# ZLkanyo009/Yolo-compression-and-deployment-in-FPGA

Measured on AMD Instinct MI355X. Metric: images/sec slim_yolo_v2 int8 416x416, higher is better.
Workload: dtype int8; 1 GPU; slim_yolo_v2_q_bf int8, batch 64 per GPU, 416x416, 2 classes, conf 0.01; global_batch=64, parallelism=batch-shard x1, streams_per_gpu=4, ring_workgroups_per_launch=128, input=f32, input_batches_rotated=4

## Files before the change

yolo-compression-and-deployment-in-fpga_amd/csrc/conv3x3_ring.hip:

```cpp
#include "y355_common.h"
#ifndef Y355_RING_XCD_SHARE
#define Y355_RING_XCD_SHARE 1
#endif
#include <type_traits>
#include <hip/hip_ext.h>
#include <cstdlib>
#ifndef Y355_DIAG
#define Y355_DIAG 0
#endif
#ifndef Y355_DIAG12
#define Y355_DIAG12 (Y355_DIAG == 1 || Y355_DIAG == 2)
#endif
#ifndef Y355_RING_PF
#define Y355_RING_PF 4
#endif

__device__ __forceinline__ void rglds16(const void *g, void *lds) {
    __builtin_amdgcn_global_load_lds((const __attribute__((address_space(1))) void *)g,
                                     (__attribute__((address_space(3))) void *)lds, 16, 0, 0);
}
template <int N>
__device__ __forceinline__ void rwait_vmcnt() {
    static_assert(N >= 0, "vmcnt");
    asm volatile("s_waitcnt vmcnt(%0)" ::"n"(N > 63 ? 63 : N) : "memory");
}

constexpr float RMAGIC = 12582912.0f, RQLO = 12582785.0f, RQHI = 12583039.0f;
__device__ __forceinline__ float rvmax(float a, float b) {
    float d;
    asm("v_max_f32 %0, %1, %2" : "=v"(d) : "v"(a), "v"(b));
    return d;
}
__device__ __forceinline__ float rvmax3(float a, float b, float c) {
    float d;
    asm("v_max3_f32 %0, %1, %2, %3" : "=v"(d) : "v"(a), "v"(b), "v"(c));
    return d;
}
__device__ __forceinline__ float rvmin3(float a, float b, float c) {
    float d;
    asm("v_min3_f32 %0, %1, %2, %3" : "=v"(d) : "v"(a), "v"(b), "v"(c));
    return d;
}
template <int B>
__device__ __forceinline__ void rmax_to_byte(unsigned int &w, float a, float b) {
    if constexpr (B == 0)
        asm("v_max_f32_sdwa %0, %1, %2 dst_sel:BYTE_0 dst_unused:UNUSED_PAD src0_sel:DWORD src1_sel:DWORD" : "=v"(w) : "v"(a), "v"(b));
    else if constexpr (B == 1)
        asm("v_max_f32_sdwa %0, %1, %2 dst_sel:BYTE_1 dst_unused:UNUSED_PRESERVE src0_sel:DWORD src1_sel:DWORD" : "+v"(w) : "v"(a), "v"(b));
    else if constexpr (B == 2)
        asm("v_max_f32_sdwa %0, %1, %2 dst_sel:BYTE_2 dst_unused:UNUSED_PRESERVE src0_sel:DWORD src1_sel:DWORD" : "+v"(w) : "v"(a), "v"(b));
    else
        asm("v_max_f32_sdwa %0, %1, %2 dst_sel:BYTE_3 dst_unused:UNUSED_PRESERVE src0_sel:DWORD src1_sel:DWORD" : "+v"(w) : "v"(a), "v"(b));
}
__device__ __forceinline__ unsigned int rpack4(float a, float b, float c, float d) {
    const unsigned int ab = __builtin_amdgcn_perm(__float_as_uint(b), __float_as_uint(a), 0x0c0c0400u);
    const unsigned int cd = __builtin_amdgcn_perm(__float_as_uint(d), __float_as_uint(c), 0x04000c0cu);
    return ab | cd;
}

__device__ __forceinline__ void rwait_vmcnt_dyn(int n) {
#define RW_CASE(k) case k: asm volatile("s_waitcnt vmcnt(" #k ")" ::: "memory"); break;
    switch (n < 0 ? 0 : (n > 63 ? 63 : n)) {
        RW_CASE(0) RW_CASE(1) RW_CASE(2) RW_CASE(3) RW_CASE(4) RW_CASE(5) RW_CASE(6) RW_CASE(7) RW_CASE(8) RW_CASE(9)
        RW_CASE(10) RW_CASE(11) RW_CASE(12) RW_CASE(13) RW_CASE(14) RW_CASE(15) RW_CASE(16) RW_CASE(17) RW_CASE(18)
        RW_CASE(19) RW_CASE(20) RW_CASE(21) RW_CASE(22) RW_CASE(23) RW_CASE(24) RW_CASE(25) RW_CASE(26) RW_CASE(27)
        RW_CASE(28) RW_CASE(29) RW_CASE(30) RW_CASE(31) RW_CASE(32) RW_CASE(33) RW_CASE(34) RW_CASE(35) RW_CASE(36)
        RW_CASE(37) RW_CASE(38) RW_CASE(39) RW_CASE(40) RW_CASE(41) RW_CASE(42) RW_CASE(43) RW_CASE(44) RW_CASE(45)
        RW_CASE(46) RW_CASE(47) RW_CASE(48) RW_CASE(49) RW_CASE(50) RW_CASE(51) RW_CASE(52) RW_CASE(53) RW_CASE(54)
        RW_CASE(55) RW_CASE(56) RW_CASE(57) RW_CASE(58) RW_CASE(59) RW_CASE(60) RW_CASE(61) RW_CASE(62) RW_CASE(63)
    }
#undef RW_CASE
}

constexpr int ring_sp(int lo, int hi, int ppw, bool prev) {
    int n = 0;
    for (int u = lo; u <= hi; ++u) {
        if (u < 0 && !prev) continue;
        const int t = ((u % 9) + 9) % 9;
        if (t >= 1 && t <= ppw) ++n;
    }
    return n;
}

template <int CIN, int BN, int TH, int TW, bool POOL, int WM, int WN, int PF, bool ROLL, bool DIRECT_REQ, bool FPE = false>
__global__ __launch_bounds__(WM * WN * 64, (WM * WN == 4) ? 2 : 1) void conv3x3_i8_ring_kernel(const ConvParams p, const int total_tiles) {
    constexpr int NW = WM * WN;
    constexpr int NTHR = NW * 64;
    constexpr int NCH = CIN / 64, SPC = 9, KS = NCH * SPC;
    constexpr int PW = TW + 2, PH = TH + 2;
    constexpr int PWL = (PW + 7) / 8 * 8;
    constexpr int NPIX = PH * PWL;
    constexpr int BM = TH * TW;
    constexpr int MT_TOT = (BM + 15) / 16;
    constexpr int MT = (MT_TOT + WM - 1) / WM;
    constexpr int NT = BN / 16 / WN;
    constexpr int SLABB = (NPIX * 64 + 1023) / 1024 * 1024;
    constexpr int NPIECE = SLABB / 1024;
    constexpr int PPW = (NPIECE + NW - 1) / NW;
    constexpr int WB = (BN / 16) * 1024;
    constexpr int NFR = BN / 16;
    constexpr int WPW = (NFR + NW - 1) / NW;
    constexpr int WSLOTS = PF + 2;
    constexpr int OFF_W = 2 * SLABB;
    constexpr int OFF_DUMMY = OFF_W + WSLOTS * WB;
    constexpr int OFF_BIAS = OFF_DUMMY + 1024;
    constexpr int SROWS = POOL ? MT * WM * 4 : MT * WM * 16;
    constexpr int SSTR = BN + 16;
    constexpr int OROWS = POOL ? BM / 4 : BM;
    constexpr bool DIRECT = DIRECT_REQ && (SROWS * SSTR > SLABB);
    constexpr int NPASS = (!DIRECT && SROWS * SSTR > SLABB) ? 2 : 1;
    constexpr int RP = SROWS / NPASS;
    constexpr int CG = BN / 16;
    constexpr int NITP = (RP * CG + NTHR - 1) / NTHR;
    constexpr int NIT = DIRECT ? (POOL ? MT : MT * 4) : NPASS * NITP;
    static_assert(CIN % 64 == 0 && NT == 4, "64-channel chunks, four n-tiles per wave");
    static_assert(PPW <= 8 && PF >= 2 && PF <= 8, "slab pieces go out at t = 1..PPW");
    static_assert(!(FPE && (DIRECT_REQ || ROLL)), "the fp32 epilogue is written for the staged path and the unrolled chunk loop");
    static_assert(DIRECT || (RP * SSTR <= SLABB && MT % NPASS == 0), "staging fits the dead slot");
    constexpr int UNRC = ROLL ? 1 : NCH;
    constexpr bool STATIC = !ROLL && KS % WSLOTS == 0 && NCH % 2 == 0;
    extern __shared__ __attribute__((aligned(16))) char smem[];

    const int tid = threadIdx.x;
    const int lane = tid & 63;
    const int wave = __builtin_amdgcn_readfirstlane(tid >> 6);
    const int wm = wave / WN, wn = wave % WN;
    const int li = lane & 15, g = lane >> 4;
    const int H = p.H, W = p.W;

    static_assert((NW * 16) % PWL == 0 && NPIX % 16 == 0, "slab pieces step by whole patch rows");
    constexpr int PSTEP = NW * 16 / PWL;
    const int pix0 = wave * 16 + (lane >> 2);
    const int ppy0 = pix0 / PWL, ppx0 = min(pix0 % PWL, PW - 1);
    const int pwithin = ((lane & 3) ^ ((lane >> 3) & 3)) << 4;
    auto decode = [&](int tile, int &b, int &y0, int &x0, int &nb) {
        if (p.xcd_share_log2 > 0) {
            const int gs = 8 << p.xcd_share_log2;
            if (tile < (total_tiles & ~(gs - 1))) {
                const int j = tile & (gs - 1);
                tile = (tile & ~(gs - 1)) | ((j & 7) << p.xcd_share_log2) | (j >> 3);
            }
        }
        nb = tile % p.nblk;
        tile /= p.nblk;
        x0 = (tile % p.tiles_x) * TW;
        tile /= p.tiles_x;
        y0 = (tile % p.tiles_y) * TH;
        b = tile / p.tiles_y;
    };
    auto issue_slab_piece = [&](int b, int y0, int x0, int c, int slot, int j) {
        const int q = wave + NW * j;
        const int8_t *inb = p.in + (size_t)b * (H + 2) * (W + 2) * CIN + c * 64;
        const int gy = min(y0 + ppy0 + j * PSTEP, H + 1), gx = min(x0 + ppx0, W + 1);
        const int8_t *src = inb + ((size_t)gy * (W + 2) + gx) * CIN + pwithin;
        char *dst = (q < NPIECE) ? smem + slot * SLABB + q * 1024 : smem + OFF_DUMMY;
        rglds16(src, dst);
    };
    auto issue_w = [&](int nb, int ks, int slot) {
#pragma unroll
        for (int j = 0; j < WPW; ++j) {
            const int f = wave + NW * j;
            const bool ok = NFR % NW == 0 || f < NFR;
            const int8_t *src = p.w + ((size_t)(nb * KS + ks) * NFR + (ok ? f : 0)) * 1024 + lane * 16;
            char *dst = ok ? smem + OFF_W + slot * WB + f * 1024 : smem + OFF_DUMMY;
            rglds16(src, dst);
        }
    };
    auto wrap = [](int s) { return s >= WSLOTS ? s - WSLOTS : s; };
// ... 39 lines not shown
    for (int k = 0; k <= PF; ++k) {
        if (k < KS) issue_w(nb, k, k);
        else issue_w(nb, k - KS, k);
    }
    pstamp(1);
    const Requant rq = p.rq;
    unsigned int nsat = 0;
    bool first = true;

    for (;;) {
        int ntile = tile + gridDim.x;
        const bool more = ntile < total_tiles;
        if (!more) ntile = tile;
        int b2, y2, x2, nb2;
        decode(ntile, b2, y2, x2, nb2);
        int abase[MT][3];
        {
            int li_a = li, g_a = g;
            asm volatile("" : "+v"(li_a), "+v"(g_a));
#pragma unroll
            for (int m = 0; m < MT; ++m) {
                int row = (wm * MT + m) * 16 + li_a;
                row = min(row, BM - 1);
                int oy, ox;
                if constexpr (POOL) {
                    const int w = row >> 2, r = row & 3;
                    oy = 2 * (w / (TW / 2)) + (r >> 1);
                    ox = 2 * (w % (TW / 2)) + (r & 1);
                } else {
                    oy = row / TW;
                    ox = row % TW;
                }
#pragma unroll
                for (int dx = 0; dx < 3; ++dx)
                    abase[m][dx] = (oy * PWL + ox + dx) * 64 + ((g_a ^ (((ox + dx) >> 1) & 3)) << 4);
            }
        }

        v4i acc[MT][NT];
        if constexpr (!FPE) {
#pragma unroll
            for (int m = 0; m < MT; ++m)
#pragma unroll
                for (int t = 0; t < NT; ++t) acc[m][t] = (v4i){0, 0, 0, 0};
        }

        v4i bfb[2][NT];
        v4i afp[2];
        if (first) rwait_vmcnt<PF * WPW>();
        else rwait_vmcnt<PF * WPW + ring_sp(-PF, -1, PPW, true) + NIT>();
        __builtin_amdgcn_s_barrier();
        pstamp(first ? 2 : 6);
        if constexpr (FPE) {
            const v4i bv = *(const v4i *)(smem + OFF_BIAS + (nb * BN + wn * (NT * 16) + li * NT) * 4);
#pragma unroll
            for (int m = 0; m < MT; ++m)
#pragma unroll
                for (int t = 0; t < NT; ++t) acc[m][t] = (v4i){bv[t], bv[t], bv[t], bv[t]};
        }
        {
            const char *wb0 = smem + OFF_W + (STATIC ? 0 : wq) * WB + (wn * NT) * 1024 + lane * 16;
#pragma unroll
            for (int tt = 0; tt < NT; ++tt) bfb[0][tt] = *(const v4i *)(wb0 + tt * 1024);
        }
#pragma unroll UNRC
        for (int c = 0; c < NCH; ++c) {
            const int slc = STATIC ? (c & 1) : sl;
            const int soff = slc * SLABB;
            const bool lastc = (c + 1 == NCH);
#pragma unroll
            for (int t = 0; t < SPC; ++t) {
                const int s_idx = c * SPC + t;
                {
                    constexpr int n_slab = (9 - PPW) * WPW;
                    const bool fine = Y355_DIAG12 && first && c == (NCH > 1 ? 1 : 0);
                    if (fine) stamp();
                    if constexpr (ROLL) {
                        const int n0f = (PF - 1) * WPW + ring_sp(t - PF + 1, t - 1, PPW, false);
                        int n0l = (PF - 1) * WPW + ring_sp(t - PF + 1, t - 1, PPW, true) + (t < PF ? NIT : 0);
                        int nr = (PF - 1) * WPW + ring_sp(9 + t - PF + 1, 9 + t - 1, PPW, true);
                        if (t == 0) {
                            if (n_slab + NIT < n0l) n0l = n_slab + NIT;
                            if (n_slab < nr) nr = n_slab;
                        }
                        if (c == 0) {
                            if (first) rwait_vmcnt_dyn(n0f);
                            else rwait_vmcnt_dyn(n0l);
                        } else {
                            rwait_vmcnt_dyn(nr);
                        }
                    } else {
                        const int lo = s_idx - PF + 1, hi = s_idx - 1;
                        int n_first = (PF - 1) * WPW + ring_sp(lo, hi, PPW, false);
                        int n_later = (PF - 1) * WPW + ring_sp(lo, hi, PPW, true) + (s_idx < PF ? NIT : 0);
                        if (t == 0) {
                            if (c > 0 && n_slab < n_first) n_first = n_slab;
                            const int n_slab2 = n_slab + (c == 0 ? NIT : 0);
                            if (n_slab2 < n_later) n_later = n_slab2;
                        }
                        if (n_first == n_later) rwait_vmcnt_dyn(n_later);
                        else if (first) rwait_vmcnt_dyn(n_first);
                        else rwait_vmcnt_dyn(n_later);
                    }
                    if (fine) stamp();
                }
                __builtin_amdgcn_s_barrier();
                if (Y355_DIAG12 && first && c == (NCH > 1 ? 1 : 0)) stamp();
// ... 142 lines not shown
                            }
                            const int qq = y355_requant_fast(v, bias[t], rq);
                            const int q = y355_clamp8<int>(qq);
                            nsat += (srow < OROWS && oy0 + srow / OTW < Ho && ox0 + srow % OTW < Wo && q != qq) ? 1u : 0u;
                            w |= (unsigned int)(q & 0xff) << (8 * t);
                        }
                        const int oy = oy0 + srow / OTW, ox = ox0 + srow % OTW;
                        int8_t *dst = outb + ((size_t)(oy + halo) * (Wo + 2 * halo) + ox + halo) * p.cstride + ncol;
                        if (!(srow < OROWS && oy < Ho && ox < Wo)) dst = p.sink + tid * 4;
                        *(unsigned int *)dst = w;
                        __builtin_amdgcn_sched_barrier(0);
                    }
            } else {
            asm volatile("s_waitcnt lgkmcnt(0)" ::: "memory");
            __builtin_amdgcn_s_barrier();
#pragma unroll
            for (int ps = 0; ps < NPASS; ++ps) {
                if (ps > 0) {
                    asm volatile("s_waitcnt lgkmcnt(0)" ::: "memory");
                    __builtin_amdgcn_s_barrier();
                }
                constexpr int MH = MT / NPASS;
                constexpr int RPMT = POOL ? 4 : 16;
                auto stage = [&](auto clampc) {
                    constexpr bool CL = decltype(clampc)::value;
#pragma unroll
                    for (int mm = 0; mm < MH; ++mm) {
                        const int m = ps * MH + mm;
#pragma unroll
                        for (int r = 0; r < RPM; ++r) {
                            const int lrow = POOL ? (wm * MH + mm) * 4 + g : (wm * MH + mm) * 16 + 4 * g + r;
                            unsigned int w = 0;
                            float yq[NT], ypos[NT], yneg[NT];
#pragma unroll
                            for (int t = 0; t < NT; ++t) {
                                int v;
                                if constexpr (POOL) {
                                    const v4i a = acc[m][t];
                                    v = max(max(a[0], a[1]), max(a[2], a[3]));
                                } else {
                                    v = acc[m][t][r];
                                }
                                if constexpr (FPE) {
                                    if constexpr (CL) asm volatile("" : "+v"(v));
                                    yq[t] = requantf(v, t, ypos[t], yneg[t]);
                                } else {
                                    const int qq = requant(v, t);
                                    const int q = y355_clamp8<int>(qq);
                                    satx += (unsigned int)(q ^ qq);
                                    w |= (unsigned int)(q & 0xff) << (8 * t);
                                }
                            }
                            if constexpr (FPE) {
                                static_assert(!FPE || NT == 4, "the fp32 epilogue packs four channels per lane and row");
                                if constexpr (CL) {
                                    float yc[NT];
#pragma unroll
                                    for (int t = 0; t < NT; ++t) yc[t] = __builtin_amdgcn_fmed3f(rvmax(ypos[t], yneg[t]), RQLO, RQHI);
                                    w = rpack4(yc[0], yc[1], yc[2], yc[3]);
                                } else {
                                    ymx = rvmax3(rvmax3(ymx, ypos[0], ypos[1]), ypos[2], ypos[3]);
                                    ymn = rvmin3(rvmin3(ymn, yneg[0], yneg[1]), yneg[2], yneg[3]);
                                    rmax_to_byte<0>(w, ypos[0], yneg[0]);
                                    rmax_to_byte<1>(w, ypos[1], yneg[1]);
                                    rmax_to_byte<2>(w, ypos[2], yneg[2]);
                                    rmax_to_byte<3>(w, ypos[3], yneg[3]);
                                }
                            }
                            *(unsigned int *)(stg + lrow * SSTR + ncol) = w;
                            if constexpr (FPE) __builtin_amdgcn_sched_barrier(0);
                        }
                    }
                };
                stage(std::false_type{});
                if constexpr (FPE) {
                    if (__builtin_amdgcn_ballot_w64(ymx > RQHI || ymn < RQLO) != 0ull) stage(std::true_type{});
                }
                if (Y355_DIAG12 && first) stamp();
                asm volatile("s_waitcnt lgkmcnt(0)" ::: "memory");
                __builtin_amdgcn_s_barrier();
                if (Y355_DIAG12 && first) stamp();
#pragma unroll
                for (int j = 0; j < NITP; ++j) {
                    const int it = min(tid + j * NTHR, RP * CG - 1);
                    const int rl = it / CG, cg = it % CG;
                    const int row = ((rl / (MH * RPMT)) * MT + ps * MH) * RPMT + rl % (MH * RPMT);
                    const int oy = oy0 + row / OTW, ox = ox0 + row % OTW;
                    const v4i v = *(const v4i *)(stg + rl * SSTR + cg * 16);
                    int8_t *dst = outb + ((size_t)(oy + halo) * (Wo + 2 * halo) + ox + halo) * p.cstride + cg * 16;
                    if (!(row < OROWS && oy < Ho && ox < Wo)) dst = p.sink + tid * 16;
                    *(v4i *)dst = v;
                }
            }
            if constexpr (FPE) satx = (ymx > RQHI || ymn < RQLO) ? 1u : 0u;
            if (satx) {
#pragma unroll
                for (int m = 0; m < MT; ++m)
#pragma unroll
                    for (int r = 0; r < RPM; ++r) {
                        const int srow = POOL ? (wm * MT + m) * 4 + g : (wm * MT + m) * 16 + 4 * g + r;
                        const bool real = srow < OROWS && oy0 + srow / OTW < Ho && ox0 + srow % OTW < Wo;
#pragma unroll
                        for (int t = 0; t < NT; ++t) {
                            int v;
                            if constexpr (POOL) {
                                const v4i a = acc[m][t];
                                v = max(max(a[0], a[1]), max(a[2], a[3]));
                            } else {
                                v = acc[m][t][r];
                            }
                            if constexpr (FPE) {
                                asm volatile("" : "+v"(v));
                                float ypc, ync;
                                (void)requantf(v, t, ypc, ync);
                                const float y = rvmax(ypc, ync);
                                nsat += (real && (y > RQHI || y < RQLO)) ? 1u : 0u;
                            } else {
                                const int qq = requant(v, t);
                                nsat += (real && y355_clamp8<int>(qq) != qq) ? 1u : 0u;
                            }
                        }
                    }
// ... 11 lines not shown
    pstamp(5);
    if (Y355_DIAG12) { nstamp = 28; stamp(); }
    if (nsat) atomicAdd(&p.ctr->sat, (unsigned long long)nsat);
}

template <int CIN, int BN, int TH, int TW, bool POOL, int WM, int WN, int PF, bool ROLL, bool DIRECT, bool FPE>
struct ConvInstR {
    static constexpr int PWL = (TW + 2 + 7) / 8 * 8;
    static constexpr int SLABB = ((TH + 2) * PWL * 64 + 1023) / 1024 * 1024;
    static constexpr int WB = (BN / 16) * 1024;
    static constexpr size_t LDS = 2 * (size_t)SLABB + (size_t)(PF + 2) * WB + 1024 + (FPE ? 1024 : 0);
    static int prepare() {
        return (int)hipFuncSetAttribute((const void *)conv3x3_i8_ring_kernel<CIN, BN, TH, TW, POOL, WM, WN, PF, ROLL, DIRECT, FPE>,
                                        hipFuncAttributeMaxDynamicSharedMemorySize, (int)LDS);
    }
    static bool launch(const ConvParams &p_in, hipStream_t s) {
        ConvParams p = p_in;
        p.tiles_x = (p.W + TW - 1) / TW;
        p.tiles_y = (p.H + TH - 1) / TH;
        const int total = p.tiles_x * p.tiles_y * p.nblk * p.B;
        {
            const int per_image = p.tiles_x * p.tiles_y * p.nblk;
            p.xcd_share_log2 = !Y355_RING_XCD_SHARE ? 0 : (per_image == 8 && WM * WN == 4) ? 3 : per_image == 4 ? 2 : (per_image == 2 || p.nblk == 2) ? 1 : 0;
        }
        constexpr int PER_CU = (WM * WN == 4) ? 2 : 1;
        int grid = y355_cu_count() * PER_CU;
        if (p.grid_limit > 0 && p.grid_limit * PER_CU < grid) grid = p.grid_limit * PER_CU;
        if (grid > total) grid = total;
        if (p.ev_start && p.ev_stop) {
            hipEvent_t e0 = (hipEvent_t)p.ev_start, e1 = (hipEvent_t)p.ev_stop;
            p.ev_start = p.ev_stop = nullptr;
            hipExtLaunchKernelGGL((conv3x3_i8_ring_kernel<CIN, BN, TH, TW, POOL, WM, WN, PF, ROLL, DIRECT, FPE>), dim3(grid), dim3(WM * WN * 64), LDS, s,
                                  e0, e1, 0, p, total);
        } else {
            hipLaunchKernelGGL((conv3x3_i8_ring_kernel<CIN, BN, TH, TW, POOL, WM, WN, PF, ROLL, DIRECT, FPE>), dim3(grid), dim3(WM * WN * 64), LDS, s, p, total);
        }
        return true;
    }
};

template <bool ROLL, bool DIRECT, bool FPE>
struct RSet {
    using C3_2 = ConvInstR<64, 64, 26, 26, true, 8, 1, Y355_RING_PF, ROLL, DIRECT, FPE>;
    using C4_1 = ConvInstR<64, 128, 13, 26, false, 4, 2, Y355_RING_PF, ROLL, DIRECT, FPE>;
    using C4_2 = ConvInstR<128, 64, 26, 26, true, 8, 1, Y355_RING_PF, ROLL, DIRECT, FPE>;
    using C5 = ConvInstR<128, 128, 13, 26, false, 4, 2, Y355_RING_PF, ROLL, DIRECT, FPE>;
#if Y355_RING_C67_SMALL
    using C67 = ConvInstR<256, 128, 13, 13, false, 2, 2, Y355_RING_PF, ROLL, DIRECT, FPE>;
#else
    using C67 = ConvInstR<256, 128, 13, 26, false, 4, 2, Y355_RING_PF, ROLL, DIRECT, FPE>;
#endif
    using PRED = ConvInstR<256, 64, 13, 13, false, 8, 1, Y355_RING_PF, ROLL, DIRECT, FPE>;
    using PRED_W = ConvInstR<256, 64, 13, 26, false, 8, 1, Y355_RING_PF, ROLL, DIRECT, FPE>;
    static int prepare() {
        int e = C3_2::prepare();
        if (!e) e = C4_1::prepare();
        if (!e) e = C4_2::prepare();
        if (!e) e = C5::prepare();
        if (!e) e = C67::prepare();
        if (!e) e = PRED::prepare();
        if (!e) e = PRED_W::prepare();
        return e;
    }
    static bool launch(int kid, const ConvParams &p, hipStream_t s) {
        switch (kid) {
        case Y355_K_CONV3_2: return C3_2::launch(p, s);
        case Y355_K_CONV4_1: return C4_1::launch(p, s);
        case Y355_K_CONV4_2: return C4_2::launch(p, s);
        case Y355_K_CONV5: return C5::launch(p, s);
        case Y355_K_CONV67: return C67::launch(p, s);
        case Y355_K_PRED: return p.grid_limit > 0 ? PRED_W::launch(p, s) : PRED::launch(p, s);
        default: return false;
        }
    }
};

int y355_prepare_conv_ring(void) {
    const int e = RSet<false, false, false>::prepare();
    return e ? e : RSet<false, false, true>::prepare();
}

bool y355_launch_conv_ring(int kid, const ConvParams &p, hipStream_t s) {
    if ((p.mode & 0xff) != 0 || p.rq.wide || p.guard) return false;
#ifndef Y355_RING_NO_FPE
    if (p.rq.shl == 0 && p.rq.sh_l == 0 && p.rq.sh_r <= 17 && p.rq.neg_mul == 1 && p.cstride >= 4 && p.cstride <= 256)
        return RSet<false, false, true>::launch(kid, p, s);
#endif
    return RSet<false, false, false>::launch(kid, p, s);
}
```

yolo-compression-and-deployment-in-fpga_amd/csrc/engine.hip:

```cpp
#include "../../include/yolo355.h"
#include "y355_common.h"

#include <algorithm>
#include <cmath>
#include <cstdio>
#include <cstdlib>
#include <cstring>
#include <string>
#include <vector>

static thread_local std::string g_err;
int y355_fail(int code, const std::string &msg) {
    g_err = msg;
    return code;
}
static int fail(int code, const std::string &msg) { return y355_fail(code, msg); }
#define HIPCHK(expr)                                                                      \
    do {                                                                                  \
        hipError_t e_ = (expr);                                                           \
        if (e_ != hipSuccess)                                                             \
            return fail(Y355_EHIP, std::string(#expr) + ": " + hipGetErrorString(e_));    \
    } while (0)

extern "C" const char *y355_last_error(void) { return g_err.c_str(); }
extern "C" int y355_version(void) { return 2; }

#ifndef Y355_GL_TAB
#define Y355_GL_TAB {100, 100, 100, 100, 100, 100, 100, 100, 100, 100}
#endif
static const int kGridLimitPct[10] = Y355_GL_TAB;
#ifndef Y355_TPUT_PAIRS_WGS
#define Y355_TPUT_PAIRS_WGS 1
#endif
namespace {
struct LayerDef { int cin, cout, pool, leaky, kid; };
const LayerDef kLayers[10] = {
    {3, 16, 1, 1, -1},
    {16, 32, 1, 1, Y355_K_CONV2},
    {32, 64, 0, 1, Y355_K_CONV3_1},
    {64, 64, 1, 1, Y355_K_CONV3_2},
    {64, 128, 0, 1, Y355_K_CONV4_1},
    {128, 128, 1, 1, Y355_K_CONV4_2},
    {128, 256, 0, 1, Y355_K_CONV5},
    {256, 256, 0, 1, Y355_K_CONV67},
    {256, 256, 0, 1, Y355_K_CONV67},
    {256, 0, 0, 0, Y355_K_PRED},
};
const int kRetuneDefault[10] = {11, 10, 10, 11, 11, 10, 11, 11, 11, 10};

struct Layer {
    int cin = 0, cout = 0, cout_pad = 0, pool = 0, leaky = 0, kid = -1;
    int Hin = 0, Win = 0, Hout = 0, Wout = 0, halo = 1;
    int e_w = 0, e_b = 0;
    bool loaded = false, bias_dirty = true;
    std::vector<int32_t> q_b;
    int8_t *w_dev = nullptr;
    int8_t *wpx_dev = nullptr;
    long long wabs = 0;
    int *bias_dev = nullptr;
    long long *bias_w_dev = nullptr;
    int8_t *out_dev = nullptr;
    size_t out_bytes = 0;
    Requant rq{};
    int frac_bits = 0;
};

int kernels_prepared = 0;
}
int y355_prepare_kernels() {
    if (kernels_prepared) return 0;
    for (int i = 0; i < Y355_K_COUNT; ++i) {
        int e = y355_conv_kernel(i)->prepare();
        if (e) return fail(Y355_EHIP, std::string("hipFuncSetAttribute: ") + hipGetErrorString((hipError_t)e));
    }
    if (int e = y355_prepare_head())
        return fail(Y355_EHIP, std::string("hipFuncSetAttribute(head): ") + hipGetErrorString((hipError_t)e));
    if (int e = y355_prepare_conv_ring())
        return fail(Y355_EHIP, std::string("hipFuncSetAttribute(ring): ") + hipGetErrorString((hipError_t)e));
    if (int e = y355_prepare_pair3())
        return fail(Y355_EHIP, std::string("hipFuncSetAttribute(pair3): ") + hipGetErrorString((hipError_t)e));
    if (int e = y355_prepare_conv_px())
        return fail(Y355_EHIP, std::string("hipFuncSetAttribute(px): ") + hipGetErrorString((hipError_t)e));
    if (int e = y355_prepare_convg())
        return fail(Y355_EHIP, std::string("hipFuncSetAttribute(convg): ") + hipGetErrorString((hipError_t)e));
    kernels_prepared = 1;
    return 0;
}
int y355_cu_count(void) {
    static int cached[64] = {};
    int dev = 0;
    if (hipGetDevice(&dev) != hipSuccess || dev < 0 || dev >= 64) return 256;
    if (!cached[dev]) {
        int n = 0;
        if (hipDeviceGetAttribute(&n, hipDeviceAttributeMultiprocessorCount, dev) != hipSuccess || n <= 0) n = 256;
        cached[dev] = n;
    }
    return cached[dev];
}
namespace {
int prepare_kernels() { return y355_prepare_kernels(); }

int make_requant(int cin_real, int taps, int sa_in, int e_w, int e_b, int sa_out, bool have_out, int act, int retune,
                 const int32_t *q_b, int cout, int cout_pad, Requant *rq, int *frac_bits, std::vector<int32_t> *bias_t,
                 std::vector<long long> *bias_w, long long wabs = 0) {
    const int F = std::max(sa_in + e_w, e_b);
    const int shl = F - sa_in - e_w, bshl = F - e_b;
    const int leaky = act == 1 ? 1 : 0;
    const int Fp = F + (leaky ? 3 : 0);
    if (shl > 30 || bshl > 40) return fail(Y355_ERANGE, "exponent gap too large for the fixed-point epilogue");
    long long bmax = 0;
// ... 44 lines not shown
}
}

int y355_op_requant(int cin, int taps, int sa_in, int e_w, int e_b, int act, const int32_t *q_b, int cout, int cout_pad, Requant *rq,
                    int *frac_bits, std::vector<int32_t> *bias_t, std::vector<long long> *bias_w) {
    return make_requant(cin, taps, sa_in, e_w, e_b, 0, false, act, 10, q_b, cout, cout_pad, rq, frac_bits, bias_t, bias_w);
}

struct y355_engine {
    y355_config cfg{};
    hipStream_t stream = nullptr;
    bool own_stream = false;
    Layer L[10];
    int sa[11];
    bool sa_set[11];
    int retune[10];
    float trk_scale[11] = {};
    int trk_first[11] = {};
    float nmean[3] = {0.485f, 0.456f, 0.406f};
    float nstd[3] = {0.229f, 0.224f, 0.225f};
    const uint8_t *x_u8 = nullptr;
    uint8_t *rs_frames = nullptr;
    int *rs_tab = nullptr;
    int rs_src_h = 0, rs_src_w = 0;
    int8_t *w0_dev = nullptr;
    int8_t *wf_dev = nullptr;
    Counters *ctr_dev = nullptr;
    CounterSets ctrs;
    unsigned int *absmax_dev = nullptr;
    int8_t *sink_dev = nullptr;
    unsigned long long *stamps_dev = nullptr;
    int Hs = 0, Ws = 0, N = 0;
    y355_head_ws ws{};
    float *cand_box = nullptr, *cand_score = nullptr;
    int *cand_cls = nullptr;
    float *x_stage = nullptr;
    float *o_box = nullptr, *o_score = nullptr;
    int *o_cls = nullptr, *o_count = nullptr;
    int max_det = 0;
    int stamp_layer = -1;
    int profile = 0;
    int fuse_front = 1;
    int fuse_pairs = 1;
    int l2_batch = 0;
    int l0_batch = 0;
    int ring_wgs = 0;
    hipEvent_t ev[Y355_NUM_TIMERS + 1];
    hipEvent_t kev[Y355_NUM_KERNEL_TIMERS][2];
    bool kev_set[Y355_NUM_KERNEL_TIMERS] = {};
    bool ev_ok = false;
    std::vector<void *> allocs;
};

static int dmalloc(y355_engine *h, void **p, size_t bytes, bool zero) {
    HIPCHK(hipMalloc(p, bytes ? bytes : 16));
    h->allocs.push_back(*p);
    if (zero) HIPCHK(hipMemset(*p, 0, bytes ? bytes : 16));
    return 0;
}

extern "C" void y355_destroy(y355_engine *h) {
    if (!h) return;
    (void)hipSetDevice(h->cfg.device_id);
    if (h->stream) (void)hipStreamSynchronize(h->stream);
    for (void *p : h->allocs) (void)hipFree(p);
    if (h->ev_ok) {
        for (auto &e : h->ev) (void)hipEventDestroy(e);
        for (auto &e : h->kev) { (void)hipEventDestroy(e[0]); (void)hipEventDestroy(e[1]); }
    }
    if (h->own_stream && h->stream) (void)hipStreamDestroy(h->stream);
    delete h;
}

extern "C" int y355_create(const y355_config *cfg, y355_engine **out) {
    if (!cfg || !out) return fail(Y355_EINVAL, "null argument");
    if (cfg->height <= 0 || cfg->width <= 0 || cfg->height % 16 || cfg->width % 16)
        return fail(Y355_EINVAL, "input size must be a positive multiple of 16");
    if (cfg->num_anchors < 1 || cfg->num_anchors > Y355_MAX_ANCHORS || cfg->num_classes < 1)
        return fail(Y355_EINVAL, "bad anchors / classes");
    if (cfg->max_batch < 1) return fail(Y355_EINVAL, "max_batch < 1");
    const int predc = cfg->num_anchors * (5 + cfg->num_classes);
    if (predc > 256) return fail(Y355_EINVAL, "A*(5+C) > 256 not supported");
    const int Hs = cfg->height / 16, Ws = cfg->width / 16, N = Hs * Ws * cfg->num_anchors;
    if (N > Y355_NMS_CAP) return fail(Y355_EINVAL, "more than 4096 anchors per image not supported");
    HIPCHK(hipSetDevice(cfg->device_id));
    if (int e = prepare_kernels()) return e;
    y355_engine *h = new y355_engine();
    h->cfg = *cfg;
    h->Hs = Hs;
    h->Ws = Ws;
    h->N = N;
    h->max_det = (cfg->max_det <= 0 || cfg->max_det > N) ? N : cfg->max_det;
    for (int i = 0; i < 11; ++i) { h->sa[i] = 0; h->sa_set[i] = false; }
    for (int i = 0; i < 10; ++i) h->retune[i] = kRetuneDefault[i];
    if (!cfg->own_stream) {
        h->stream = (hipStream_t)cfg->stream;
    } else {
        if (hipStreamCreateWithFlags(&h->stream, hipStreamNonBlocking) != hipSuccess) {
            delete h;
            return fail(Y355_EHIP, "hipStreamCreate failed");
        }
        h->own_stream = true;
    }
    const int B = cfg->max_batch;
    int Hc = cfg->height, Wc = cfg->width;
    int rc = 0;
    for (int k = 0; k < 10 && !rc; ++k) {
        Layer &L = h->L[k];
        const LayerDef &d = kLayers[k];
        L.cin = d.cin;
        L.cout = d.cout ? d.cout : predc;
        L.pool = d.pool;
        L.leaky = d.leaky;
        L.kid = d.kid;
        L.Hin = Hc;
        L.Win = Wc;
        L.Hout = d.pool ? Hc / 2 : Hc;
        L.Wout = d.pool ? Wc / 2 : Wc;
        L.halo = (k == 9) ? 0 : 1;
        if (k == 0) L.cout_pad = 16;
        else {
            const int bn = y355_conv_kernel(L.kid)->bn;
            L.cout_pad = (L.cout + bn - 1) / bn * bn;
        }
        L.out_bytes = ((size_t)B * (L.Hout + 2 * L.halo) * (L.Wout + 2 * L.halo) + 64) * L.cout_pad;
        rc = dmalloc(h, (void **)&L.out_dev, L.out_bytes, true);
        if (!rc) rc = dmalloc(h, (void **)&L.bias_dev, sizeof(int) * L.cout_pad, true);
        if (!rc) rc = dmalloc(h, (void **)&L.bias_w_dev, sizeof(long long) * L.cout_pad, true);
        if (!rc && k > 0) rc = dmalloc(h, (void **)&L.w_dev, y355_packed_bytes(*y355_conv_kernel(L.kid), L.cout_pad), true);
        Hc = L.Hout;
        Wc = L.Wout;
    }
    const size_t cap = Y355_NMS_CAP;
    if (!rc) rc = dmalloc(h, (void **)&h->w0_dev, 1024, true);
    if (!rc) rc = dmalloc(h, (void **)&h->wf_dev, 16384, true);
    if (!rc) rc = dmalloc(h, (void **)&h->ctr_dev, sizeof(Counters) * 20, true);
    h->ctrs.base = h->ctr_dev;
    h->ctrs.n = 10;
    h->ctrs.clean[0] = h->ctrs.clean[1] = true;
    if (!rc) rc = dmalloc(h, (void **)&h->absmax_dev, 16, true);
    if (!rc) rc = dmalloc(h, (void **)&h->sink_dev, 16384, true);
    if (!rc) rc = dmalloc(h, &h->ws.cbox, sizeof(float) * 4 * cap * B, false);
    if (!rc) rc = dmalloc(h, &h->ws.cscore, sizeof(float) * cap * B, false);
    if (!rc) rc = dmalloc(h, &h->ws.ccls, sizeof(int) * cap * B, false);
    if (!rc) rc = dmalloc(h, &h->ws.corig, sizeof(int) * cap * B, false);
    if (!rc) rc = dmalloc(h, &h->ws.count, sizeof(int) * B, true);
    if (!rc) rc = dmalloc(h, &h->ws.edges, sizeof(unsigned int) * (size_t)Y355_HEAD_EDGE_CAP * B, false);
    if (!rc) rc = dmalloc(h, &h->ws.nedges, sizeof(int) * 2 * (size_t)B, true);
    if (!rc) rc = dmalloc(h, &h->ws.binstart, sizeof(int) * (cap + 8) * B, true);
    if (!rc) rc = dmalloc(h, &h->ws.astat, sizeof(float) * 4 * Y355_HEAD_MAXG * B, true);
    if (!rc) rc = dmalloc(h, &h->ws.tiny, sizeof(int) * cap * B, true);
    if (!rc) rc = dmalloc(h, &h->ws.ntiny, sizeof(int) * B, true);
    if (!rc) rc = dmalloc(h, &h->ws.dbox, sizeof(float) * 4 * cap * B, true);
    if (!rc) rc = dmalloc(h, &h->ws.dscore, sizeof(float) * cap * B, true);
    if (!rc) rc = dmalloc(h, &h->ws.dcls, sizeof(int) * cap * B, true);
    if (!rc) rc = dmalloc(h, &h->ws.ctype, sizeof(int) * cap * B, true);
    if (!rc) rc = dmalloc(h, (void **)&h->cand_box, sizeof(float) * 4 * N * B, false);
    if (!rc) rc = dmalloc(h, (void **)&h->cand_score, sizeof(float) * N * B, false);
    if (!rc) rc = dmalloc(h, (void **)&h->cand_cls, sizeof(int) * N * B, false);
    if (!rc) rc = dmalloc(h, (void **)&h->o_box, sizeof(float) * 4 * h->max_det * B, false);
    if (!rc) rc = dmalloc(h, (void **)&h->o_score, sizeof(float) * h->max_det * B, false);
    if (!rc) rc = dmalloc(h, (void **)&h->o_cls, sizeof(int) * h->max_det * B, false);
    if (!rc) rc = dmalloc(h, (void **)&h->o_count, sizeof(int) * B, true);
    if (!rc) {
        bool ok = true;
        for (auto &e : h->ev) ok = ok && (hipEventCreate(&e) == hipSuccess);
        for (auto &e : h->kev) ok = ok && (hipEventCreate(&e[0]) == hipSuccess) && (hipEventCreate(&e[1]) == hipSuccess);
        h->ev_ok = ok;
        if (!ok) rc = fail(Y355_EHIP, "hipEventCreate failed");
    }
    if (rc) {
        std::string keep = g_err;
        y355_destroy(h);
        g_err = keep;
        return rc;
    }
    *out = h;
    return 0;
}

extern "C" int y355_set_option(y355_engine *h, int option, int value) {
    if (!h) return fail(Y355_EINVAL, "null engine");
    switch (option) {
    case Y355_OPT_FUSE_FRONT:
        if (value != 0 && value != 1) return fail(Y355_EINVAL, "Y355_OPT_FUSE_FRONT takes 0 or 1");
        h->fuse_front = value;
        return 0;
    case Y355_OPT_FUSE_PAIRS:
        if (value != 0 && value != 1) return fail(Y355_EINVAL, "Y355_OPT_FUSE_PAIRS takes 0 or 1");
        h->fuse_pairs = value;
        return 0;
    case Y355_OPT_RING_WORKGROUPS:
        if (value < 0 || value > 4096) return fail(Y355_EINVAL, "workgroups per launch out of range");
        h->ring_wgs = value;
        return 0;
    default: return fail(Y355_EINVAL, "unknown option");
    }
}

extern "C" int y355_set_thresholds(y355_engine *h, float conf, float nms) {
    if (!h) return fail(Y355_EINVAL, "null engine");
    h->cfg.conf_thresh = conf;
    h->cfg.nms_thresh = nms;
    return 0;
}

extern "C" int y355_load_layer(y355_engine *h, int idx, const int8_t *q_w, const int32_t *q_b, int cout, int cin,
                               int e_w, int e_b) {
    if (!h || !q_w || !q_b) return fail(Y355_EINVAL, "null argument");
    if (idx < 0 || idx >= 10) return fail(Y355_EINVAL, "layer index out of range");
    Layer &L = h->L[idx];
    if (cout != L.cout || cin != L.cin) {
        char buf[128];
        snprintf(buf, sizeof buf, "layer %d expects [%d,%d,3,3], got [%d,%d,3,3]", idx, L.cout, L.cin, cout, cin);
        return fail(Y355_EINVAL, buf);
    }
    HIPCHK(hipSetDevice(h->cfg.device_id));
    HIPCHK(hipStreamSynchronize(h->stream));
    if (idx == 0) {
        int8_t frag[1024];
        y355_pack_conv1(q_w, frag);
        HIPCHK(hipMemcpy(h->w0_dev, frag, 1024, hipMemcpyHostToDevice));
        std::vector<int8_t> ff(16384);
        y355_pack_front(q_w, nullptr, ff.data());
        HIPCHK(hipMemcpy(h->wf_dev, ff.data(), 4096, hipMemcpyHostToDevice));
    } else {
        const ConvKernelInfo &ki = *y355_conv_kernel(L.kid);
        std::vector<int8_t> packed(y355_packed_bytes(ki, L.cout_pad));
        y355_pack_weights(ki, q_w, cout, cin, L.cout_pad, packed.data());
        HIPCHK(hipMemcpy(L.w_dev, packed.data(), packed.size(), hipMemcpyHostToDevice));
        if (idx == 1) {
            std::vector<int8_t> ff(16384);
            y355_pack_front(nullptr, q_w, ff.data());
            HIPCHK(hipMemcpy(h->wf_dev + 4096, ff.data() + 4096, 12288, hipMemcpyHostToDevice));
        }
    }
    {
        long long best = 0;
        const size_t per = (size_t)cin * 9;
        for (int c = 0; c < cout; ++c) {
            long long sum = 0;
            for (size_t i = 0; i < per; ++i) sum += std::abs((int)q_w[(size_t)c * per + i]);
            best = std::max(best, sum);
        }
        L.wabs = best;
    }
    if (const size_t pxb = idx > 0 ? y355_px_packed_bytes(L.kid) : 0) {
        std::vector<int8_t> px(pxb);
        if (y355_pack_px(L.kid, q_w, cout, cin, px.data())) {
            if (!L.wpx_dev) {
                if (int rc = dmalloc(h, (void **)&L.wpx_dev, px.size(), false)) return rc;
            }
            HIPCHK(hipMemcpy(L.wpx_dev, px.data(), px.size(), hipMemcpyHostToDevice));
        }
    }
    L.q_b.assign(q_b, q_b + cout);
    L.e_w = e_w;
    L.e_b = e_b;
    L.loaded = true;
    L.bias_dirty = true;
    return 0;
}

extern "C" int y355_set_act_exponents(y355_engine *h, const int32_t *sa) {
    if (!h || !sa) return fail(Y355_EINVAL, "null argument");
    for (int i = 0; i < 11; ++i)
        if (sa[i] < -64 || sa[i] > 64) return fail(Y355_EINVAL, "activation exponent out of range");
    for (int i = 0; i < 11; ++i) {
        if (h->sa_set[i] && h->sa[i] == sa[i]) continue;
        h->sa[i] = sa[i];
        h->sa_set[i] = true;
        if (i < 10) h->L[i].bias_dirty = true;
        if (i > 0) h->L[i - 1].bias_dirty = true;
    }
    return 0;
}

static int set_one_exponent(y355_engine *h, int i, int v) {
    if (h->sa_set[i] && h->sa[i] == v) return 0;
    h->sa[i] = v;
    h->sa_set[i] = true;
    if (i < 10) h->L[i].bias_dirty = true;
    if (i > 0) h->L[i - 1].bias_dirty = true;
// ... 52 lines not shown
        p.bias_w = L.bias_w_dev;
        p.ctr = h->ctr_dev;
        p.B = B;
        p.H = L.Hin;
        p.W = L.Win;
        y355_conv1_tiles(L.Hin, L.Win, &p.tiles_x, &p.tiles_y);
        p.in_scale = std::ldexp(1.0f, h->sa[0]);
        p.rq = L.rq;
        p.mode = mode;
        p.guard = guard;
        y355_launch_conv1(p, h->stream);
        if (mode == 0) h->l0_batch = B;
    } else {
        const ConvKernelInfo &ki = *y355_conv_kernel(L.kid);
        ConvParams p{};
        p.in = h->L[k - 1].out_dev;
        p.out = L.out_dev;
        p.w = L.w_dev;
        p.bias_t = L.bias_dev;
        p.bias_w = L.bias_w_dev;
        p.ctr = h->ctr_dev + k;
        p.sink = h->sink_dev;
        p.stamps = (h->stamp_layer == k) ? h->stamps_dev : nullptr;
        h->kev_set[k] = false;
        if (h->profile == 2 && mode == 0) { p.ev_start = h->kev[k][0]; p.ev_stop = h->kev[k][1]; }
        p.grid_limit = h->ring_wgs * kGridLimitPct[k] / 100;
        p.B = B;
        p.H = L.Hin;
        p.W = L.Win;
        p.cstride = L.cout_pad;
        p.out_halo = L.halo;
        p.tiles_x = (L.Win + ki.tw - 1) / ki.tw;
        p.tiles_y = (L.Hin + ki.th - 1) / ki.th;
        p.nblk = L.cout_pad / ki.bn;
        p.rq = L.rq;
        p.mode = mode;
        p.guard = guard;
#ifdef Y355_EXPERIMENTS
        static const int no_ring_mask = getenv("Y355_NO_RING_MASK") ? atoi(getenv("Y355_NO_RING_MASK")) : 0;
        static const int no_px_mask = getenv("Y355_NO_PX_MASK") ? atoi(getenv("Y355_NO_PX_MASK")) : 0;
#else
        constexpr int no_ring_mask = 0, no_px_mask = 0;
#endif
        if (k == 2 && mode == 0) h->l2_batch = B;
        if (L.wpx_dev && !((no_px_mask >> k) & 1)) {
            ConvParams q = p;
            q.w = L.wpx_dev;
            if (y355_launch_conv_px(L.kid, q, h->stream)) {
                HIPCHK(hipGetLastError());
                h->kev_set[k] = p.ev_start != nullptr;
                return 0;
            }
        }
        if (!((no_ring_mask >> k) & 1) && y355_launch_conv_ring(L.kid, p, h->stream)) {
            HIPCHK(hipGetLastError());
            h->kev_set[k] = p.ev_start != nullptr;
            return 0;
        }
        ki.launch(p, p.tiles_x * p.tiles_y * p.nblk * B, h->stream);
    }
    HIPCHK(hipGetLastError());
    return 0;
}

extern "C" int y355_input_absmax(y355_engine *h, const float *x_dev, int batch, float *out_max) {
    if (!h || !x_dev || !out_max) return fail(Y355_EINVAL, "null argument");
    if (batch < 1 || batch > h->cfg.max_batch) return fail(Y355_EINVAL, "batch out of range");
    HIPCHK(hipSetDevice(h->cfg.device_id));
    HIPCHK(hipMemsetAsync(h->absmax_dev, 0, 16, h->stream));
    y355_launch_absmax(x_dev, (size_t)batch * 3 * h->cfg.height * h->cfg.width, h->absmax_dev, h->stream);
    HIPCHK(hipGetLastError());
    unsigned int bits = 0;
    HIPCHK(hipMemcpyAsync(&bits, h->absmax_dev, 4, hipMemcpyDeviceToHost, h->stream));
    HIPCHK(hipStreamSynchronize(h->stream));
    memcpy(out_max, &bits, 4);
    return 0;
}

extern "C" int y355_run_layer(y355_engine *h, int idx, int batch, int mode, const float *x_dev) {
    if (!h) return fail(Y355_EINVAL, "null engine");
    if (idx < 0 || idx >= 10 || (mode != 0 && mode != 1)) return fail(Y355_EINVAL, "bad layer / mode");
    if (batch < 1 || batch > h->cfg.max_batch) return fail(Y355_EINVAL, "batch out of range");
    if (idx == 0 && !x_dev) return fail(Y355_EINVAL, "layer 0 needs the network input");
    HIPCHK(hipSetDevice(h->cfg.device_id));
    if (int rc = refresh_layer(h, idx, mode == 0)) return rc;
    HIPCHK(hipMemsetAsync(h->ctr_dev + idx, 0, sizeof(Counters), h->stream));
    return launch_layer(h, idx, batch, mode, 1, x_dev);
}

extern "C" int y355_layer_stats_get(y355_engine *h, int idx, y355_layer_stats *out) {
    if (!h || !out || idx < 0 || idx >= 10) return fail(Y355_EINVAL, "bad argument");
    HIPCHK(hipSetDevice(h->cfg.device_id));
    Counters c;
    HIPCHK(hipMemcpyAsync(&c, h->ctr_dev + idx, sizeof c, hipMemcpyDeviceToHost, h->stream));
    HIPCHK(hipStreamSynchronize(h->stream));
    out->absmax_t = (int64_t)c.absmax;
    out->frac_bits = h->L[idx].frac_bits;
    out->reserved = (int32_t)c.in_sat;
    out->saturated = (int64_t)c.sat + (idx == 0 ? c.in_sat : 0);
    out->guard = (int64_t)c.guard;
    return 0;
}

static int tracker_update(float *scale, int *first, int i, float max_abs, int freeze, double momentum, int *exp_out) {
    const float s = (1.0f / max_abs) * 127.0f;
    if (!*first) {
        *first = 1;
        *scale = *scale + s;
    } else if (!freeze) {
        const float keep = (float)(1.0 - momentum), mom = (float)momentum;
// ... 644 lines not shown
```

yolo-compression-and-deployment-in-fpga_amd/csrc/y355_common.h:

```cpp
#pragma once
#include <hip/hip_runtime.h>
#include <stdint.h>

#include <hip/hip_ext.h>

typedef int v4i __attribute__((ext_vector_type(4)));
#define Y355_STAMP_ROWS 4096

#define Y355_LAUNCH(kernel, grid, block, lds, stream, e0, e1, ...)                                                       \
    do {                                                                                                                 \
        if ((e0) && (e1)) hipExtLaunchKernelGGL(kernel, grid, block, lds, stream, (hipEvent_t)(e0), (hipEvent_t)(e1), 0, __VA_ARGS__); \
        else hipLaunchKernelGGL(kernel, grid, block, lds, stream, __VA_ARGS__);                                          \
    } while (0)

struct Requant {
    int shl;
    int sh;
    int leaky;
    int guard_log2;
    int wide;
    int lk, sh_l, sh_r, hm1, bw;
    int neg_mul;
    int gen32;
    int tmax_log2;
// ... 30 lines not shown
    int t = (acc << rq.shl) + bias;
    t = max(t, t << rq.lk);
    const int rb = (int)__builtin_amdgcn_ubfe((unsigned int)t, (unsigned int)rq.sh_r, (unsigned int)rq.bw);
    return ((t << rq.sh_l) + rq.hm1 + rb) >> rq.sh_r;
}

struct Counters {
    unsigned long long absmax;
    unsigned long long in_sat;
    unsigned long long sat;
    unsigned long long guard;
};

int y355_cu_count(void);
int y355_zero_counters(Counters *c, int n, hipStream_t s);

struct CounterSets {
    Counters *base = nullptr;
    int n = 0, cur = 0;
    bool clean[2] = {false, false};
    Counters *set(int i) const { return base + (size_t)i * n; }
    Counters *begin(bool *need_zero) {
        cur ^= 1;
        *need_zero = !clean[cur];
        clean[cur] = false;
        return set(cur);
    }
    Counters *other_zeroed_by_front() {
        clean[cur ^ 1] = true;
        return set(cur ^ 1);
    }
};

struct ConvParams {
    const int8_t *in;
    int8_t *out;
    const int8_t *w;
    const int *bias_t;
    const long long *bias_w;
    Counters *ctr;
    int8_t *sink;
    long long *raw;
    unsigned long long *stamps;
    int B, H, W;
    int cstride;
    int out_halo;
    int tiles_x, tiles_y, nblk;
    Requant rq;
    int mode;
    int guard;
    void *ev_start, *ev_stop;
    int grid_limit;
    int xcd_share_log2;
};

struct Conv1Params {
    const float *x;
    const uint8_t *x_u8;
    float nmean[3], nstd[3];
    int8_t *out;
    int out_pb;
    const int8_t *w;
    const int *bias_t;
    const long long *bias_w;
    const int *shl_c;
    Counters *ctr;
    int B, H, W;
    int tiles_x, tiles_y;
    float in_scale;
    Requant rq;
    int mode;
    int guard;
};

struct FrontParams {
    const float *x;
    const uint8_t *x_u8;
    float nmean[3], nstd[3];
    int8_t *out;
    const int8_t *wf;
    const int *bias1;
    const int *bias2;
    Counters *ctr;
    unsigned long long *zero_next;
    int zero_n;
    int B, H, W;
    int tiles_x, tiles_y;
    float in_scale;
    float in_thr;
    int step_x, step_y, step_b;
    Requant rq1, rq2;
    unsigned long long *stamps;
    void *ev_start, *ev_stop;
};
struct FrontBParams {
    const float *x;
    const uint8_t *x_u8;
    float nmean[3], nstd[3];
    char *out;
    int out_pb;
    const char *wf;
    const float *bias1;
    const float *bias2;
    int B, H, W;
    int tiles_x, tiles_y;
    float slope1, slope2;
// ... 283 lines not shown
```

Before: 318,600 images/sec.

## Use narrower ring kernel for prediction conv with small output channel count

The prediction conv layer has few output channels (2 classes, about 35 channels), but the ring kernel always computed a 64-wide N tile. This adds ring kernel instantiations with BN of 32 or 48 (one to three n-tiles per wave) plus a separately packed weight buffer sized to that width, and routes the pred layer to them. The goal is to skip the MFMA work and weight traffic spent on padded channels. The cost is more template instances and a generalized epilogue for NT below four.

```diff
diff --git a/yolo-compression-and-deployment-in-fpga_amd/csrc/conv3x3_ring.hip b/yolo-compression-and-deployment-in-fpga_amd/csrc/conv3x3_ring.hip
--- a/yolo-compression-and-deployment-in-fpga_amd/csrc/conv3x3_ring.hip
+++ b/yolo-compression-and-deployment-in-fpga_amd/csrc/conv3x3_ring.hip
@@ -40,6 +40,22 @@
     float d;
     asm("v_min3_f32 %0, %1, %2, %3" : "=v"(d) : "v"(a), "v"(b), "v"(c));
     return d;
+}
+__device__ __forceinline__ float rvmin(float a, float b) {
+    float d;
+    asm("v_min_f32 %0, %1, %2" : "=v"(d) : "v"(a), "v"(b));
+    return d;
+}
+template <int NT>
+__device__ __forceinline__ void rstore_nt(void *dst, unsigned int w) {
+    if constexpr (NT == 4) {
+        *(unsigned int *)dst = w;
+    } else if constexpr (NT == 2) {
+        *(unsigned short *)dst = (unsigned short)w;
+    } else {
+#pragma unroll
+        for (int t = 0; t < NT; ++t) ((unsigned char *)dst)[t] = (unsigned char)(w >> (8 * t));
+    }
 }
 template <int B>
 __device__ __forceinline__ void rmax_to_byte(unsigned int &w, float a, float b) {
@@ -113,7 +129,8 @@
     constexpr int CG = BN / 16;
     constexpr int NITP = (RP * CG + NTHR - 1) / NTHR;
     constexpr int NIT = DIRECT ? (POOL ? MT : MT * 4) : NPASS * NITP;
-    static_assert(CIN % 64 == 0 && NT == 4, "64-channel chunks, four n-tiles per wave");
+    static_assert(CIN % 64 == 0 && NT >= 1 && NT <= 4, "64-channel chunks, one to four n-tiles per wave (pred: ceil(cout / 16))");
+    static_assert(NT == 4 || !DIRECT_REQ, "the direct epilogue stores four channels per lane");
     static_assert(PPW <= 8 && PF >= 2 && PF <= 8, "slab pieces go out at t = 1..PPW");
     static_assert(!(FPE && (DIRECT_REQ || ROLL)), "the fp32 epilogue is written for the staged path and the unrolled chunk loop");
     static_assert(DIRECT || (RP * SSTR <= SLABB && MT % NPASS == 0), "staging fits the dead slot");
@@ -259,7 +276,18 @@
         __builtin_amdgcn_s_barrier();
         pstamp(first ? 2 : 6);
         if constexpr (FPE) {
-            const v4i bv = *(const v4i *)(smem + OFF_BIAS + (nb * BN + wn * (NT * 16) + li * NT) * 4);
+            int bv[NT];
+            {
+                const char *bp = smem + OFF_BIAS + (nb * BN + wn * (NT * 16) + li * NT) * 4;
+                if constexpr (NT == 4) {
+                    const v4i v = *(const v4i *)bp;
+#pragma unroll
+                    for (int t = 0; t < NT; ++t) bv[t] = v[t];
+                } else {
+#pragma unroll
+                    for (int t = 0; t < NT; ++t) bv[t] = ((const int *)bp)[t];
+                }
+            }
 #pragma unroll
             for (int m = 0; m < MT; ++m)
 #pragma unroll
@@ -508,22 +536,28 @@
                                 }
                             }
                             if constexpr (FPE) {
-                                static_assert(!FPE || NT == 4, "the fp32 epilogue packs four channels per lane and row");
                                 if constexpr (CL) {
                                     float yc[NT];
 #pragma unroll
                                     for (int t = 0; t < NT; ++t) yc[t] = __builtin_amdgcn_fmed3f(rvmax(ypos[t], yneg[t]), RQLO, RQHI);
-                                    w = rpack4(yc[0], yc[1], yc[2], yc[3]);
+                                    w = rpack4(yc[0], yc[NT > 1 ? 1 : 0], yc[NT > 2 ? 2 : 0], yc[NT - 1]);
                                 } else {
-                                    ymx = rvmax3(rvmax3(ymx, ypos[0], ypos[1]), ypos[2], ypos[3]);
-                                    ymn = rvmin3(rvmin3(ymn, yneg[0], yneg[1]), yneg[2], yneg[3]);
+#pragma unroll
+                                    for (int t = 0; t + 1 < NT; t += 2) {
+                                        ymx = rvmax3(ymx, ypos[t], ypos[t + 1]);
+                                        ymn = rvmin3(ymn, yneg[t], yneg[t + 1]);
+                                    }
+                                    if constexpr (NT % 2) {
+                                        ymx = rvmax(ymx, ypos[NT - 1]);
+                                        ymn = rvmin(ymn, yneg[NT - 1]);
+                                    }
                                     rmax_to_byte<0>(w, ypos[0], yneg[0]);
-                                    rmax_to_byte<1>(w, ypos[1], yneg[1]);
-                                    rmax_to_byte<2>(w, ypos[2], yneg[2]);
-                                    rmax_to_byte<3>(w, ypos[3], yneg[3]);
+                                    if constexpr (NT > 1) rmax_to_byte<1>(w, ypos[1], yneg[1]);
+                                    if constexpr (NT > 2) rmax_to_byte<2>(w, ypos[2], yneg[2]);
+                                    if constexpr (NT > 3) rmax_to_byte<3>(w, ypos[3], yneg[3]);
                                 }
                             }
-                            *(unsigned int *)(stg + lrow * SSTR + ncol) = w;
+                            rstore_nt<NT>(stg + lrow * SSTR + ncol, w);
                             if constexpr (FPE) __builtin_amdgcn_sched_barrier(0);
                         }
                     }
@@ -641,6 +675,10 @@
 #endif
     using PRED = ConvInstR<256, 64, 13, 13, false, 8, 1, Y355_RING_PF, ROLL, DIRECT, FPE>;
     using PRED_W = ConvInstR<256, 64, 13, 26, false, 8, 1, Y355_RING_PF, ROLL, DIRECT, FPE>;
+    template <int BNR>
+    using PRED_N = ConvInstR<256, BNR, 13, 13, false, 8, 1, Y355_RING_PF, ROLL, DIRECT, FPE>;
+    template <int BNR>
+    using PRED_WN = ConvInstR<256, BNR, 13, 26, false, 8, 1, Y355_RING_PF, ROLL, DIRECT, FPE>;
     static int prepare() {
         int e = C3_2::prepare();
         if (!e) e = C4_1::prepare();
@@ -649,7 +687,19 @@
         if (!e) e = C67::prepare();
         if (!e) e = PRED::prepare();
         if (!e) e = PRED_W::prepare();
+        if (!e) e = PRED_N<32>::prepare();
+        if (!e) e = PRED_WN<32>::prepare();
+        if (!e) e = PRED_N<48>::prepare();
+        if (!e) e = PRED_WN<48>::prepare();
         return e;
+    }
+    static bool launch_pred(const ConvParams &p, hipStream_t s) {
+        const bool wide = p.grid_limit > 0;
+        switch (p.ring_bn) {
+        case 32: return wide ? PRED_WN<32>::launch(p, s) : PRED_N<32>::launch(p, s);
+        case 48: return wide ? PRED_WN<48>::launch(p, s) : PRED_N<48>::launch(p, s);
+        default: return wide ? PRED_W::launch(p, s) : PRED::launch(p, s);
+        }
     }
     static bool launch(int kid, const ConvParams &p, hipStream_t s) {
         switch (kid) {
@@ -658,7 +708,7 @@
         case Y355_K_CONV4_2: return C4_2::launch(p, s);
         case Y355_K_CONV5: return C5::launch(p, s);
         case Y355_K_CONV67: return C67::launch(p, s);
-        case Y355_K_PRED: return p.grid_limit > 0 ? PRED_W::launch(p, s) : PRED::launch(p, s);
+        case Y355_K_PRED: return launch_pred(p, s);
         default: return false;
         }
     }
diff --git a/yolo-compression-and-deployment-in-fpga_amd/csrc/engine.hip b/yolo-compression-and-deployment-in-fpga_amd/csrc/engine.hip
--- a/yolo-compression-and-deployment-in-fpga_amd/csrc/engine.hip
+++ b/yolo-compression-and-deployment-in-fpga_amd/csrc/engine.hip
@@ -56,6 +56,8 @@
     std::vector<int32_t> q_b;
     int8_t *w_dev = nullptr;
     int8_t *wpx_dev = nullptr;
+    int8_t *wring_dev = nullptr;
+    int ring_bn = 0;
     long long wabs = 0;
     int *bias_dev = nullptr;
     long long *bias_w_dev = nullptr;
@@ -206,6 +208,14 @@
     std::vector<void *> allocs;
 };
 
+static ConvKernelInfo ring_pred_info(int bn) {
+    ConvKernelInfo ki = *y355_conv_kernel(Y355_K_PRED);
+    ki.bn = bn;
+    ki.wn = 1;
+    ki.nt = bn / 16;
+    return ki;
+}
+
 static int dmalloc(y355_engine *h, void **p, size_t bytes, bool zero) {
     HIPCHK(hipMalloc(p, bytes ? bytes : 16));
     h->allocs.push_back(*p);
@@ -282,6 +292,10 @@
         if (!rc) rc = dmalloc(h, (void **)&L.bias_dev, sizeof(int) * L.cout_pad, true);
         if (!rc) rc = dmalloc(h, (void **)&L.bias_w_dev, sizeof(long long) * L.cout_pad, true);
         if (!rc && k > 0) rc = dmalloc(h, (void **)&L.w_dev, y355_packed_bytes(*y355_conv_kernel(L.kid), L.cout_pad), true);
+        if (!rc && L.kid == Y355_K_PRED && L.cout <= 48) {
+            L.ring_bn = L.cout <= 32 ? 32 : 48;
+            rc = dmalloc(h, (void **)&L.wring_dev, y355_packed_bytes(ring_pred_info(L.ring_bn), L.ring_bn), true);
+        }
         Hc = L.Hout;
         Wc = L.Wout;
     }
@@ -383,6 +397,12 @@
         std::vector<int8_t> packed(y355_packed_bytes(ki, L.cout_pad));
         y355_pack_weights(ki, q_w, cout, cin, L.cout_pad, packed.data());
         HIPCHK(hipMemcpy(L.w_dev, packed.data(), packed.size(), hipMemcpyHostToDevice));
+        if (L.wring_dev) {
+            const ConvKernelInfo kr = ring_pred_info(L.ring_bn);
+            std::vector<int8_t> pr(y355_packed_bytes(kr, L.ring_bn));
+            y355_pack_weights(kr, q_w, cout, cin, L.ring_bn, pr.data());
+            HIPCHK(hipMemcpy(L.wring_dev, pr.data(), pr.size(), hipMemcpyHostToDevice));
+        }
         if (idx == 1) {
             std::vector<int8_t> ff(16384);
             y355_pack_front(nullptr, q_w, ff.data());
@@ -541,10 +561,17 @@
                 return 0;
             }
         }
-        if (!((no_ring_mask >> k) & 1) && y355_launch_conv_ring(L.kid, p, h->stream)) {
-            HIPCHK(hipGetLastError());
-            h->kev_set[k] = p.ev_start != nullptr;
-            return 0;
+        if (!((no_ring_mask >> k) & 1)) {
+            ConvParams q = p;
+            if (L.wring_dev) {
+                q.w = L.wring_dev;
+                q.ring_bn = L.ring_bn;
+            }
+            if (y355_launch_conv_ring(L.kid, q, h->stream)) {
+                HIPCHK(hipGetLastError());
+                h->kev_set[k] = p.ev_start != nullptr;
+                return 0;
+            }
         }
         ki.launch(p, p.tiles_x * p.tiles_y * p.nblk * B, h->stream);
     }
diff --git a/yolo-compression-and-deployment-in-fpga_amd/csrc/y355_common.h b/yolo-compression-and-deployment-in-fpga_amd/csrc/y355_common.h
--- a/yolo-compression-and-deployment-in-fpga_amd/csrc/y355_common.h
+++ b/yolo-compression-and-deployment-in-fpga_amd/csrc/y355_common.h
@@ -106,6 +106,7 @@
     void *ev_start, *ev_stop;
     int grid_limit;
     int xcd_share_log2;
+    int ring_bn;
 };
 
 struct Conv1Params {
```

Result: no change. 320,500 images/sec (median of 6 runs) (+0.6%).
